# LUP-LuftbildUmweltPlanung/UNet

Hardware: AMD Instinct MI355X
Metric: 512x512 tiles/sec fwd+bwd (4-ch->5-class U-Net) (higher is better)
Workload: dtype f32

## Files before the change

### include/unet_hip.h

```cpp
#ifndef UNET_HIP_H
#define UNET_HIP_H

#include <stddef.h>
#include <stdint.h>

#ifdef __cplusplus
extern "C" {
#endif

#define UNET_OK 0
#define UNET_E_BADARG (-1)
#define UNET_E_UNSUPPORTED (-2)
#define UNET_E_HIP (-3)

#define UNET_ABI_VERSION 8

int unet_abi_version(void);
const char* unet_last_error(void);

#define UNET_F32 0
#define UNET_BF16 1
typedef uint16_t unet_bf16;

typedef struct {
    int conv_splitk;
    int mfma_shape;
    int f32_big_tile;
    int bf16_big_tile;
    int t256_tiles_per_wg;
    int t256_sliver;
    int conv1x1_gemm;
    int wgrad_mfma_shape;
    int wgrad_bf16_k4;
    int wgrad_1x1;
    int wgrad_narrow;
    int plan_batch;
    int wgrad_wgs;
    int conv_smallcin;
    int conv_head1x1;
} unet_tuning;
void unet_tuning_default(unet_tuning* t);


#define UNET_CONV_RELU 1
#define UNET_CONV_MASK 4

#define UNET_CONV_FWD 0
#define UNET_CONV_DGRAD 1

typedef struct {
    const float* x; int x_cs, x_co;
    const float* wp;
    const float* bias;
    const float* res; int res_cs, res_co;
    const float* mask; int mask_cs, mask_co;
    float* y; int y_cs, y_co;
    int N, IH, IW, Cin;
    int OH, OW, Cout;
    int ks, stride;
    int kind, flags;
    float* colsum;
    float* colsumsq;
// ... 21 lines not shown
int unet_pack_weights_bf16(const float* w, unet_bf16* wp, int Cout, int Cin, int ks, int mode, void* stream);
typedef struct {
    const float* w;
    void* wp;
    int Cout, Cin, ks, mode;
    const float* out_scale;
} unet_pack_job;
size_t unet_pack_batch_table_bytes(int njobs);
int unet_pack_batch_build(const unet_pack_job* jobs, int njobs, int dtype, void* table_host, unsigned* total_blocks);
int unet_pack_batch_run(const void* table_dev, int njobs, unsigned total_blocks, int dtype, void* stream);
typedef struct {
    const float* x; int x_cs, x_co;
    const float* dy; int dy_cs, dy_co;
    float* dw;
    float* dbias;
    int N, IH, IW, Cin, OH, OW, Cout, ks, stride;
    float* workspace; size_t workspace_floats;
    int accumulate;
    int dtype;
    const unet_tuning* tuning;
} unet_wgrad_desc;
size_t unet_conv2d_wgrad_workspace(const unet_wgrad_desc* d);
int unet_conv2d_wgrad_dma(const unet_wgrad_desc* d);
int unet_conv2d_wgrad(const unet_wgrad_desc* d, void* stream);

int unet_bn_stats_rows(long long P);
int unet_bn_stats(const float* x, int x_cs, int x_co, long long P, int C, float* partial, void* stream);
int unet_bn_finalize(const float* psum, const float* psumsq, int rows, long long count, int C,
                     const float* gamma, const float* beta, float* running_mean, float* running_var,
                     float momentum, float eps,
                     float* scale, float* shift, float* save_mean, float* save_invstd, long long* batches_tracked, void* stream);
int unet_bn_eval_coeffs(const float* gamma, const float* beta, const float* running_mean, const float* running_var,
                        float eps, int C, float* scale, float* shift, void* stream);
int unet_affine_act(const float* x, int x_cs, int x_co, const float* scale, const float* shift,
                    const float* x2, int x2_cs, int x2_co, const float* scale2, const float* shift2,
                    float* y, int y_cs, int y_co, long long P, int C, int relu, void* stream);
int unet_bn_bwd_reduce(const float* dout, int d_cs, int d_co, const float* out, int o_cs, int o_co,
                       const float* x, int x_cs, int x_co, const float* mean, const float* invstd,
                       long long P, int C, float* partial, void* stream);
int unet_bn_bwd_finalize(const float* partial, int rows, long long count, int C,
                         float* dgamma, float* dbeta, float* c1, float* c2, void* stream);
int unet_bn_bwd_apply(const float* dout, int d_cs, int d_co, const float* out, int o_cs, int o_co,
                      const float* x, int x_cs, int x_co, const float* mean, const float* invstd,
                      const float* gamma, const float* c1, const float* c2,
                      float* dx, int dx_cs, int dx_co, float* gout, int g_cs, int g_co, int g_accumulate,
                      long long P, int C, void* stream);
// ... 319 lines not shown
```

### unet_amd/_lib.py

```python
from __future__ import annotations

import ctypes as C
import os
import re
from pathlib import Path

import torch

_HERE = Path(__file__).resolve().parent
LIB_PATH = _HERE / "lib" / "libunet_hip.so"
HEADER = _HERE.parent / "include" / "unet_hip.h"

UNET_OK = 0
CONV_RELU = 1
CONV_MASK = 4
CONV_FWD = 0
CONV_DGRAD = 1
F32 = 0
BF16 = 1

c_float_p = C.POINTER(C.c_float)
vp = C.c_void_p


class Tuning(C.Structure):
    _fields_ = [(n, C.c_int) for n in ("conv_splitk", "mfma_shape", "f32_big_tile", "bf16_big_tile", "t256_tiles_per_wg", "t256_sliver",
                                       "conv1x1_gemm", "wgrad_mfma_shape", "wgrad_bf16_k4", "wgrad_1x1", "wgrad_narrow", "plan_batch", "wgrad_wgs", "conv_smallcin", "conv_head1x1")]

    @classmethod
    def default(cls, **over) -> "Tuning":
        t = cls()
        lib.unet_tuning_default(C.byref(t))
        for k, v in over.items():
            if k not in dict(cls._fields_):
                raise KeyError(f"unet_tuning has no field {k!r}")
            setattr(t, k, int(v))
        return t


class ConvDesc(C.Structure):
    _fields_ = [
        ("x", vp), ("x_cs", C.c_int), ("x_co", C.c_int),
        ("wp", vp),
        ("bias", vp),
        ("res", vp), ("res_cs", C.c_int), ("res_co", C.c_int),
        ("mask", vp), ("mask_cs", C.c_int), ("mask_co", C.c_int),
        ("y", vp), ("y_cs", C.c_int), ("y_co", C.c_int),
        ("N", C.c_int), ("IH", C.c_int), ("IW", C.c_int), ("Cin", C.c_int),
        ("OH", C.c_int), ("OW", C.c_int), ("Cout", C.c_int),
        ("ks", C.c_int), ("stride", C.c_int),
# ... 85 lines not shown


lib = _load()

i, ll, f, sz = C.c_int, C.c_longlong, C.c_float, C.c_size_t
_sig = {
    "unet_abi_version": (i, []),
    "unet_last_error": (C.c_char_p, []),
    "unet_conv2d_colsum_rows": (i, [C.POINTER(ConvDesc)]),
    "unet_conv2d": (i, [C.POINTER(ConvDesc), vp]),
    "unet_conv2d_variant": (i, [C.POINTER(ConvDesc)]),
    "unet_conv2d_splitk_workspace": (sz, [C.POINTER(ConvDesc)]),
    "unet_tuning_default": (None, [C.POINTER(Tuning)]),
    "unet_pack_batch_table_bytes": (sz, [i]),
    "unet_pack_batch_build": (i, [C.POINTER(PackJob), i, i, vp, C.POINTER(C.c_uint)]),
    "unet_pack_batch_run": (i, [vp, i, C.c_uint, i, vp]),
    "unet_pack_weights_size": (sz, [i, i, i, i]),
    "unet_pack_weights": (i, [vp, vp, i, i, i, i, vp]),
    "unet_pack_weights_strided": (i, [vp, ll, ll, vp, i, i, vp]),
    "unet_row_softmax": (i, [vp, i, i, vp, i, i, ll, i, vp]),
    "unet_row_softmax_bwd": (i, [vp, i, i, vp, i, i, vp, i, i, ll, i, vp]),
    "unet_conv2d_wgrad_workspace": (sz, [C.POINTER(WgradDesc)]),
    "unet_conv2d_wgrad_dma": (i, [C.POINTER(WgradDesc)]),
    "unet_conv2d_wgrad": (i, [C.POINTER(WgradDesc), vp]),
    "unet_bn_stats_rows": (i, [ll]),
    "unet_bn_stats": (i, [vp, i, i, ll, i, vp, vp]),
    "unet_bn_finalize": (i, [vp, vp, i, ll, i, vp, vp, vp, vp, f, f, vp, vp, vp, vp, vp, vp]),
    "unet_bn_eval_coeffs": (i, [vp, vp, vp, vp, f, i, vp, vp, vp]),
    "unet_affine_act": (i, [vp, i, i, vp, vp, vp, i, i, vp, vp, vp, i, i, ll, i, i, vp]),
    "unet_bn_bwd_reduce": (i, [vp, i, i, vp, i, i, vp, i, i, vp, vp, ll, i, vp, vp]),
    "unet_bn_bwd_finalize": (i, [vp, i, ll, i, vp, vp, vp, vp, vp]),
    "unet_bn_bwd_apply": (i, [vp, i, i, vp, i, i, vp, i, i, vp, vp, vp, vp, vp, vp, i, i, vp, i, i, i, ll, i, vp]),
    "unet_maxpool3x3s2": (i, [vp, i, i, vp, i, i, vp, i, i, i, i, i, i, vp]),
    "unet_maxpool3x3s2_bwd": (i, [vp, i, i, vp, vp, i, i, i, i, i, i, i, i, i, vp]),
    "unet_avgpool2_ceil": (i, [vp, i, i, vp, i, i, i, i, i, i, i, i, vp]),
    "unet_avgpool2_ceil_bwd": (i, [vp, i, i, vp, i, i, i, i, i, i, i, i, i, vp]),
    "unet_shuffle_blur": (i, [vp, i, i, vp, i, i, i, i, i, i, i, vp]),
    "unet_shuffle_blur_bwd": (i, [vp, i, i, vp, i, i, vp, i, i, i, i, i, i, i, vp]),
    "unet_shuffle_bwd_xmask": (i, [vp, i, i, vp, i, i, vp, i, i, i, i, i, i, vp]),
    "unet_resize_nearest": (i, [vp, i, i, vp, i, i, i, i, i, i, i, i, vp]),
    "unet_resize_nearest_bwd": (i, [vp, i, i, vp, i, i, i, i, i, i, i, i, vp]),
    "unet_nchw_to_nhwc": (i, [vp, vp, i, i, i, i, i, i, vp]),
    "unet_nhwc_to_nchw": (i, [vp, i, i, vp, i, i, i, i, vp]),
    "unet_copy_slice": (i, [vp, i, i, vp, i, i, ll, i, i, vp]),
    "unet_relu_mask": (i, [vp, i, i, vp, i, i, vp, i, i, ll, i, vp]),
    "unet_colsum": (i, [vp, i, i, ll, i, vp, vp, vp]),
# ... 146 lines not shown
```

### unet_amd/csrc/conv_dispatch.hip

```cpp
#include <stdlib.h>

#include "conv_common.h"

namespace unetconv {
static int env_int(const char* name, int dflt) {
    const char* e = getenv(name);
    return (e != nullptr && e[0] != 0) ? atoi(e) : dflt;
}
const unet_tuning& tuning_defaults() {
    static const unet_tuning t = [] {
        unet_tuning v;
        v.conv_splitk = env_int("UNET_CONV_SPLITK", 1);
        v.mfma_shape = 16;
        v.f32_big_tile = 1;
        v.bf16_big_tile = 1;
        v.t256_tiles_per_wg = 0;
        v.t256_sliver = env_int("UNET_T256_SLIVER", 1);
        v.conv1x1_gemm = env_int("UNET_CONV1X1_GEMM", 0);
        v.wgrad_mfma_shape = 32;
        v.wgrad_bf16_k4 = 1;
        v.wgrad_1x1 = 1;
        v.wgrad_narrow = 1;
        v.plan_batch = 0;
        v.wgrad_wgs = env_int("UNET_WGRAD_WGS", 0);
        v.conv_smallcin = env_int("UNET_CONV_SMALLCIN", 1);
        v.conv_head1x1 = env_int("UNET_CONV_HEAD1X1", 1);
        return v;
    }();
    return t;
}
}

extern "C" void unet_tuning_default(unet_tuning* t) {
    if (t != nullptr) *t = unetconv::tuning_defaults();
}

namespace {

using namespace unetconv;

int make_plan(const unet_conv_desc* d, Plan* p, int kc, int vec, int mf, int big_tile, int splitk, int plan_batch) {
    UNET_CHECK_ARG(d != nullptr, "conv: null desc");
    UNET_CHECK_ARG(d->x && d->wp && d->y, "conv: null tensor pointer");
    UNET_CHECK_ARG(d->ks == 1 || d->ks == 3, "conv: ks must be 1 or 3 (got %d)", d->ks);
    UNET_CHECK_ARG(d->stride == 1 || d->stride == 2, "conv: stride must be 1 or 2 (got %d)", d->stride);
    UNET_CHECK_ARG(!(d->ks == 1 && d->stride != 1), "conv: 1x1 stride 2 unsupported");
    UNET_CHECK_ARG(d->N > 0 && d->IH > 0 && d->IW > 0 && d->OH > 0 && d->OW > 0 && d->Cin > 0 && d->Cout > 0, "conv: bad dims");
    UNET_CHECK_ARG(unet::slice_ok_v(d->x_cs, d->x_co, d->Cin, vec), "conv: bad x slice cs=%d co=%d C=%d", d->x_cs, d->x_co, d->Cin);
    UNET_CHECK_ARG(unet::slice_ok_v(d->y_cs, d->y_co, d->Cout, d->y_f32 ? 4 : vec), "conv: bad y slice cs=%d co=%d C=%d", d->y_cs, d->y_co, d->Cout);
// ... 278 lines not shown
```

### unet_amd/csrc/conv_wgrad.hip

```cpp

#include <type_traits>
#include <utility>

#include "common.h"
#include "wgrad_plan.h"

namespace {

template <typename F, int... Is>
__device__ __forceinline__ void static_for_impl(F&& f, std::integer_sequence<int, Is...>) { (f(std::integral_constant<int, Is>{}), ...); }
template <int N, typename F>
__device__ __forceinline__ void static_for(F&& f) { static_for_impl(f, std::make_integer_sequence<int, N>{}); }


typedef float f32x16 __attribute__((ext_vector_type(16)));

constexpr int BK = 64;
constexpr int BC = 64;

struct WArgs {
    const float* x; const float* dy; float* part;
    float* bpart;
    int x_cs, x_co, dy_cs, dy_co;
    int N, IH, IW, Cin, Cin4, OH, OW, Cout, Cout4;
// ... 119 lines not shown
                        acc[r * KS + s] = __builtin_amdgcn_mfma_f32_32x32x2f32(av, bv, acc[r * KS + s], 0, 0, 0);
                    }
            }
            }
            __builtin_amdgcn_sched_barrier(0);
        });
        __syncthreads();
        if (has_next) store_tile();
        __syncthreads();
    }

    if (do_bias) {
        reinterpret_cast<float4*>(smem)[tid] = bq4;
        __syncthreads();
        if (tid < BK && k0 + tid < a.Cout) {
            float t = 0.f;
#pragma unroll
            for (int rr = 0; rr < 16; ++rr) t += smem[rr * 64 + tid];
            a.bpart[(size_t)split * a.Cout + k0 + tid] = t;
        }
    }
    const size_t KC_ = (size_t)a.Cout * a.Cin;
    float* pb = a.part + ((size_t)split * nsub + sub) * T * KC_;
    const int c = c0 + wc * 32 + l31;
#pragma unroll
    for (int t = 0; t < T; ++t)
#pragma unroll
        for (int r = 0; r < 16; ++r) {
            const int k = k0 + wk * 32 + (r & 3) + 8 * (r >> 2) + 4 * h;
            if (k < a.Cout && c < a.Cin) pb[(size_t)t * KC_ + (size_t)k * a.Cin + c] = acc[t][r];
        }
}

template <int PTW, int S, int KS>
__global__ __launch_bounds__(256, 2) void wgrad16_kernel(const WArgs a) {
    constexpr int PT = (S == 1) ? 64 : 32;
    constexpr int PTH = PT / PTW;
    constexpr int PAD = (KS - 1) / 2;
    constexpr int T = KS * KS;
    constexpr int HH = (PTH - 1) * S + KS, HW = (PTW - 1) * S + KS, HPIX = HH * HW;
    constexpr int DIT = (PT * 16 + 255) / 256;
    constexpr int XIT = (HPIX * 16 + 255) / 256;
    typedef float f32x4 __attribute__((ext_vector_type(4)));
    constexpr int LD = (S == 1) ? 80 : 72;

    extern __shared__ __attribute__((aligned(16))) float smem[];
// ... 938 lines not shown
        __syncthreads();
        if (tid < 128 && k0 + tid < a.Cout) {
            float t = 0.f;
#pragma unroll
            for (int rr = 0; rr < 8; ++rr) t += smem[rr * 128 + tid];
            a.bpart[(size_t)split * a.Cout + k0 + tid] = t;
        }
    }
    const size_t KC_ = (size_t)a.Cout * a.Cin;
    float* pb = a.part + (size_t)split * KC_;
#pragma unroll
    for (int i = 0; i < 2; ++i)
#pragma unroll
        for (int j = 0; j < 2; ++j) {
            const int c = c0 + wc * 64 + 32 * j + l31;
#pragma unroll
            for (int r = 0; r < 16; ++r) {
                const int k = k0 + wk * 64 + 32 * i + (r & 3) + 8 * (r >> 2) + 4 * h;
                if (k < a.Cout && c < a.Cin) pb[(size_t)k * a.Cin + c] = acc[i][j][r];
            }
        }
}

template <int K4>
__global__ __launch_bounds__(256) void wgrad1x1_small_kernel(const WArgs a, long long P, int PS, long long pix_per_block) {
    extern __shared__ __attribute__((aligned(16))) float smem[];
    const int C4 = a.Cin4 >> 2;
    const int tid = threadIdx.x;
    const int q = tid % C4, lane = tid / C4;
    const bool active = lane < PS;
    const long long p_begin = (long long)blockIdx.x * pix_per_block;
    long long p_end = p_begin + pix_per_block;
    if (p_end > P) p_end = P;
    float acc[4 * K4][4];
    float bsum[4 * K4];
#pragma unroll
    for (int k = 0; k < 4 * K4; ++k) {
        bsum[k] = 0.f;
#pragma unroll
        for (int j = 0; j < 4; ++j) acc[k][j] = 0.f;
    }
    if (active) {
        for (long long p = p_begin + lane; p < p_end; p += PS) {
            const float4 xv = *reinterpret_cast<const float4*>(a.x + (size_t)p * a.x_cs + a.x_co + 4 * q);
            const float* dyp = a.dy + (size_t)p * a.dy_cs + a.dy_co;
#pragma unroll
// ... 111 lines not shown
        const size_t t = e / KC_, i = e - t * KC_;
        float* o = dw + i * T + t;
        *o = accumulate ? (*o + s) : s;
    }
}

__global__ __launch_bounds__(256) void wgrad_bias_reduce_kernel(const float* __restrict__ bpart, float* __restrict__ dbias, int splits, int Cout) {
    __shared__ double part[4][64];
    const int cl = threadIdx.x & 63, q = threadIdx.x >> 6;
    const int c = blockIdx.x * 64 + cl;
    double s = 0.0;
    if (c < Cout)
        for (int sp = q; sp < splits; sp += 4) s += (double)bpart[(size_t)sp * Cout + c];
    part[q][cl] = s;
    __syncthreads();
    if (q == 0 && c < Cout) dbias[c] = (float)(((part[0][cl] + part[1][cl]) + part[2][cl]) + part[3][cl]);
}

struct WPlan {
    unet_tuning tune;
    WArgs k;
    int ptw, splits, T, narrow, gemm1x1, small1x1, ps, bf16;
    int dma;
    int nsub;
    long long pix_per_block;
    size_t lds_bytes, lds_bytes16;
};

int make_wplan(const unet_wgrad_desc* d, WPlan* p, bool need_dw = true) {
    UNET_CHECK_ARG(d != nullptr, "wgrad: null desc");
    p->tune = unetconv::tuning_of(d->tuning);
    UNET_CHECK_ARG(p->tune.wgrad_mfma_shape == 16 || p->tune.wgrad_mfma_shape == 32, "wgrad: unet_tuning.wgrad_mfma_shape must be 16 or 32 (start from unet_tuning_default())");
    UNET_CHECK_ARG(d->x && d->dy && (d->dw || !need_dw), "wgrad: null tensor pointer");
    UNET_CHECK_ARG(d->ks == 1 || d->ks == 3, "wgrad: ks must be 1 or 3");
    UNET_CHECK_ARG(d->stride == 1 || d->stride == 2, "wgrad: stride must be 1 or 2");
    UNET_CHECK_ARG(!(d->ks == 1 && d->stride != 1), "wgrad: 1x1 stride 2 unsupported");
    UNET_CHECK_ARG(d->N > 0 && d->IH > 0 && d->IW > 0 && d->OH > 0 && d->OW > 0 && d->Cin > 0 && d->Cout > 0, "wgrad: bad dims");
    UNET_CHECK_ARG((long long)d->N * d->OH * d->OW < (1ll << 31), "wgrad: more than 2^31 output pixels");
    const int pad = (d->ks - 1) / 2;
    UNET_CHECK_ARG(d->OH == (d->IH + 2 * pad - d->ks) / d->stride + 1 && d->OW == (d->IW + 2 * pad - d->ks) / d->stride + 1,
                   "wgrad: output dims inconsistent");
    UNET_CHECK_ARG(d->dtype == UNET_F32 || d->dtype == UNET_BF16, "wgrad: unknown dtype %d", d->dtype);
    const int vec = d->dtype == UNET_BF16 ? 8 : 4;
    p->bf16 = d->dtype == UNET_BF16;
    UNET_CHECK_ARG(unet::slice_ok_v(d->x_cs, d->x_co, d->Cin, vec), "wgrad: bad x slice");
    UNET_CHECK_ARG(unet::slice_ok_v(d->dy_cs, d->dy_co, d->Cout, vec), "wgrad: bad dy slice");
    UNET_CHECK_ARG(unet::aligned16(d->x) && unet::aligned16(d->dy), "wgrad: x/dy must be 16-byte aligned");
    WArgs& k = p->k;
    memset(&k, 0, sizeof(k));
    k.x = d->x; k.dy = d->dy; k.part = d->workspace;
    k.x_cs = d->x_cs; k.x_co = d->x_co; k.dy_cs = d->dy_cs; k.dy_co = d->dy_co;
    k.N = d->N; k.IH = d->IH; k.IW = d->IW; k.Cin = d->Cin; k.Cin4 = unet::roundup(d->Cin, vec);
    k.OH = d->OH; k.OW = d->OW; k.Cout = d->Cout; k.Cout4 = unet::roundup(d->Cout, vec);
    p->T = d->ks * d->ks;
    p->nsub = 1;
    p->dma = 0;
    p->ptw = d->OW >= 32 ? 32 : (d->OW >= 16 ? 16 : 8);
    const int pt = p->bf16 ? (d->stride == 1 ? 128 : 32) : (d->stride == 1 ? 64 : 32);
    const int pth = pt / p->ptw;
    k.tiles_y = unet::cdiv(d->OH, pth);
    k.tiles_x = unet::cdiv(d->OW, p->ptw);
    k.total_tiles = d->N * k.tiles_y * k.tiles_x;
    k.kt = unet::cdiv(d->Cout, BK);
    k.ct = unet::cdiv(d->Cin, BC);
    p->narrow = (!p->bf16 && p->tune.wgrad_narrow && d->ks == 3 && d->stride == 1 && d->Cout > 80 && d->Cout <= 112 && d->OW >= 32) ? 1 : 0;
    int cols = k.kt * k.ct;
    if (p->narrow) {
        p->ptw = 32;
        k.tiles_y = d->OH;
        k.tiles_x = unet::cdiv(d->OW, 32);
        k.total_tiles = d->N * k.tiles_y * k.tiles_x;
        const int nch = unet::cdiv(d->Cin, 112);
        k.cw = unet::roundup(unet::cdiv(d->Cin, nch), 4);
        const int ntw = d->Cout > 96 ? 5 : 7;
        k.nnb = unet::cdiv(unet::cdiv(9 * k.cw, 16), 4 * ntw);
        cols = nch * k.nnb;
        p->dma = p->tune.wgrad_narrow != 4 && flat_dma_fits(d->Cin, k.cw, k.nnb, ntw) && (long long)d->IW * d->x_cs * 4 < (1ll << 31) &&
                 (long long)d->OW * d->dy_cs * 4 < (1ll << 31);
    }
// ... 24 lines not shown
    if (p->gemm1x1) {
        k.kt = unet::cdiv(d->Cout, 128);
        k.ct = unet::cdiv(d->Cin, 128);
        k.total_tiles = unet::cdiv((long long)d->N * d->OH * d->OW, 64);
        k.tiles_y = k.tiles_x = 1;
        cols = k.kt * k.ct;
    }
    int target = 512;
    if (p->tune.wgrad_wgs > 0) target = p->tune.wgrad_wgs;
    else if (p->bf16 && d->ks == 3 && d->stride == 1 && (long long)k.total_tiles * cols <= 20000) target = 256;
    int want = target / cols;
    if ((p->narrow || p->bf16) && want >= 8) want &= ~7;
    if (want < 1) want = 1;
    int tpb = unet::cdiv(k.total_tiles, want);
    if (tpb < 4) tpb = 4;
    if (tpb > k.total_tiles) tpb = k.total_tiles;
    k.tiles_per_block = tpb;
    p->splits = unet::cdiv(k.total_tiles, tpb);
    if (!p->bf16 && !p->narrow && !p->gemm1x1 && p->tune.wgrad_mfma_shape == 32 && p->tune.wgrad_narrow != 3) {
        k.csub = d->Cin <= 32 ? 1 : 0;
        k.ksub = d->Cout <= 32 ? 1 : 0;
        p->nsub = (1 + k.csub) * (1 + k.ksub);
    }
    const int hh = (pth - 1) * d->stride + d->ks, hw = (p->ptw - 1) * d->stride + d->ks;
    p->lds_bytes = (size_t)(pt * BK + hh * hw * BC) * sizeof(float);
    p->lds_bytes16 = (size_t)(pt + hh * hw) * (d->stride == 1 ? 80 : 72) * sizeof(float);
    if (p->bf16) p->lds_bytes = (size_t)pt * 160 + (size_t)hh * hw * (d->stride == 1 ? 160 : 144);
    return UNET_OK;
}


template <int PTW, int S, int KS>
int launch_w16(const WPlan& p, hipStream_t st) {
    auto kern = wgrad16_kernel<PTW, S, KS>;
    static unsigned long long configured = 0;
    if (unet::first_use_on_device(&configured)) {
        UNET_CHECK_HIP(hipFuncSetAttribute((const void*)kern, hipFuncAttributeMaxDynamicSharedMemorySize, 160 * 1024));
    }
    hipLaunchKernelGGL(kern, dim3(p.k.kt * p.k.ct, p.splits), dim3(256), p.lds_bytes16, st, p.k);
    UNET_CHECK_LAUNCH();
    return UNET_OK;
}

template <int PTW, int S, int KS>
int launch_w(const WPlan& p, hipStream_t st) {
    if (p.tune.wgrad_mfma_shape == 16) return launch_w16<PTW, S, KS>(p, st);
// ... 59 lines not shown
    if (stride == 1) return launch_wb<PTW, 1, 3>(p, st);
    return launch_wb<PTW, 2, 3>(p, st);
}

template <int PTW>
int launch_w_ptw(const WPlan& p, int ks, int stride, hipStream_t st) {
    if (ks == 1) return launch_w<PTW, 1, 1>(p, st);
    if (stride == 1) return launch_w<PTW, 1, 3>(p, st);
    return launch_w<PTW, 2, 3>(p, st);
}

}

extern "C" size_t unet_conv2d_wgrad_workspace(const unet_wgrad_desc* d) {
    WPlan p;
    if (make_wplan(d, &p) != UNET_OK) return 0;
    return (size_t)p.splits * p.nsub * p.T * d->Cout * d->Cin + (size_t)p.splits * d->Cout;
}

extern "C" int unet_conv2d_wgrad_dma(const unet_wgrad_desc* d) {
    WPlan p;
    if (make_wplan(d, &p, false) != UNET_OK) return -1;
    return p.dma;
}

extern "C" int unet_conv2d_wgrad(const unet_wgrad_desc* d, void* stream) {
    WPlan p;
    int rc = make_wplan(d, &p);
    if (rc != UNET_OK) return rc;
    const size_t npart = (size_t)p.splits * p.nsub * p.T * d->Cout * d->Cin;
    const size_t need = npart + (size_t)p.splits * d->Cout;
    UNET_CHECK_ARG(d->workspace != nullptr && d->workspace_floats >= need, "wgrad: workspace too small (%zu < %zu floats)",
                   d->workspace_floats, need);
    p.k.bpart = d->dbias != nullptr ? d->workspace + npart : nullptr;
    hipStream_t st = (hipStream_t)stream;
    if (p.bf16) {
        switch (p.ptw) {
            case 32: rc = launch_wb_ptw<32>(p, d->ks, d->stride, st); break;
            case 16: rc = launch_wb_ptw<16>(p, d->ks, d->stride, st); break;
            default: rc = launch_wb_ptw<8>(p, d->ks, d->stride, st); break;
        }
    } else if (p.small1x1) {
        const long long P = (long long)d->N * d->OH * d->OW;
        const dim3 grid((unsigned)p.splits);
        const int k4 = (d->Cout + 3) / 4;
        const size_t lds = (size_t)p.ps * (4 * k4 * p.k.Cin4 + 4 * k4) * sizeof(float);
        UNET_CHECK_ARG(lds <= 64 * 1024, "wgrad: head kernel needs %zu bytes of LDS", lds);
        switch (k4) {
            case 1: hipLaunchKernelGGL(wgrad1x1_small_kernel<1>, grid, dim3(256), lds, st, p.k, P, p.ps, p.pix_per_block); break;
            case 2: hipLaunchKernelGGL(wgrad1x1_small_kernel<2>, grid, dim3(256), lds, st, p.k, P, p.ps, p.pix_per_block); break;
            case 3: hipLaunchKernelGGL(wgrad1x1_small_kernel<3>, grid, dim3(256), lds, st, p.k, P, p.ps, p.pix_per_block); break;
            default: hipLaunchKernelGGL(wgrad1x1_small_kernel<4>, grid, dim3(256), lds, st, p.k, P, p.ps, p.pix_per_block); break;
        }
        UNET_CHECK_LAUNCH();
        rc = UNET_OK;
    } else if (p.gemm1x1) {
        static unsigned long long configured = 0;
        if (unet::first_use_on_device(&configured)) {
            UNET_CHECK_HIP(hipFuncSetAttribute((const void*)wgrad1x1_kernel, hipFuncAttributeMaxDynamicSharedMemorySize, 160 * 1024));
        }
        hipLaunchKernelGGL(wgrad1x1_kernel, dim3(p.k.kt * p.k.ct, p.splits), dim3(256), (size_t)2 * 64 * 128 * sizeof(float), st, p.k,
                           (long long)d->N * d->OH * d->OW);
        UNET_CHECK_LAUNCH();
        rc = UNET_OK;
    } else if (p.narrow) {
        const size_t lds = p.dma ? (size_t)(2 * 32 * 112 + 3 * 15 * 256) * sizeof(float)
                                 : (size_t)(32 + 3 * 34) * 112 * sizeof(float) + (size_t)4 * 256 * 16;
        const dim3 grid(unet::cdiv(d->Cin, p.k.cw) * p.k.nnb, unet::roundup(p.splits, 8));
        static unsigned long long configured = 0;
        if (unet::first_use_on_device(&configured)) {
            UNET_CHECK_HIP(hipFuncSetAttribute((const void*)wgrad_flat_kernel<7, 5>, hipFuncAttributeMaxDynamicSharedMemorySize, 160 * 1024));
            UNET_CHECK_HIP(hipFuncSetAttribute((const void*)wgrad_flat_kernel<6, 5, true>, hipFuncAttributeMaxDynamicSharedMemorySize, 160 * 1024));
            UNET_CHECK_HIP(hipFuncSetAttribute((const void*)wgrad_flat_kernel<6, 7>, hipFuncAttributeMaxDynamicSharedMemorySize, 160 * 1024));
            UNET_CHECK_HIP(hipFuncSetAttribute((const void*)wgrad_flat_kernel<7, 5, false, true>, hipFuncAttributeMaxDynamicSharedMemorySize, 160 * 1024));
            UNET_CHECK_HIP(hipFuncSetAttribute((const void*)wgrad_flat_kernel<6, 5, true, true>, hipFuncAttributeMaxDynamicSharedMemorySize, 160 * 1024));
            UNET_CHECK_HIP(hipFuncSetAttribute((const void*)wgrad_flat_kernel<6, 7, false, true>, hipFuncAttributeMaxDynamicSharedMemorySize, 160 * 1024));
        }
        const bool sliver = d->Cout > 96 && d->Cout <= 100 && p.tune.wgrad_narrow != 2;
        if (p.dma) {
            if (sliver) hipLaunchKernelGGL((wgrad_flat_kernel<6, 5, true, true>), grid, dim3(256), lds, st, p.k);
            else if (d->Cout > 96) hipLaunchKernelGGL((wgrad_flat_kernel<7, 5, false, true>), grid, dim3(256), lds, st, p.k);
            else hipLaunchKernelGGL((wgrad_flat_kernel<6, 7, false, true>), grid, dim3(256), lds, st, p.k);
        } else if (sliver) hipLaunchKernelGGL((wgrad_flat_kernel<6, 5, true>), grid, dim3(256), lds, st, p.k);
        else if (d->Cout > 96) hipLaunchKernelGGL((wgrad_flat_kernel<7, 5>), grid, dim3(256), lds, st, p.k);
        else hipLaunchKernelGGL((wgrad_flat_kernel<6, 7>), grid, dim3(256), lds, st, p.k);
        UNET_CHECK_LAUNCH();
        rc = UNET_OK;
    } else
    switch (p.ptw) {
        case 32: rc = launch_w_ptw<32>(p, d->ks, d->stride, st); break;
        case 16: rc = launch_w_ptw<16>(p, d->ks, d->stride, st); break;
        default: rc = launch_w_ptw<8>(p, d->ks, d->stride, st); break;
    }
    if (rc != UNET_OK) return rc;
    const size_t KC_ = (size_t)d->Cout * d->Cin;
    const int slices = p.splits * p.nsub;
    if (p.small1x1)
        hipLaunchKernelGGL(wgrad_reduce_rows_kernel, dim3(unet::cdiv((int)(KC_ * p.T), 64)), dim3(256), 0, st, d->workspace, d->dw,
                           p.splits, p.T, KC_, d->accumulate);
    else if (slices >= 32 && KC_ * p.T < ((size_t)1 << 31) / 8)
        hipLaunchKernelGGL(wgrad_reduce_q_kernel<8>, dim3((unsigned)unet::cdiv((long long)(KC_ * p.T), 32LL)), dim3(256), 0, st, d->workspace, d->dw,
                           slices, p.T, KC_, d->accumulate);
    else if (slices >= 8 && KC_ * p.T < ((size_t)1 << 31) / 8)
        hipLaunchKernelGGL(wgrad_reduce_q_kernel<4>, dim3((unsigned)unet::cdiv((long long)(KC_ * p.T), 64LL)), dim3(256), 0, st, d->workspace, d->dw,
                           slices, p.T, KC_, d->accumulate);
    else
        hipLaunchKernelGGL(wgrad_reduce_kernel, dim3(unet::ew_grid((long long)KC_ * p.T, 256)), dim3(256), 0, st, d->workspace, d->dw,
                           slices, p.T, KC_, d->accumulate);
// ... 9 lines not shown
```

### unet_amd/csrc/wgrad_plan.h

```cpp
#pragma once

inline bool flat_dma_fits(int Cin, int cw, int nnb, int ntw) {
    const int nch = (Cin + cw - 1) / cw;
    const int widths[2] = {nch > 1 ? cw : Cin, Cin - (nch - 1) * cw};
    for (int CW : widths)
        for (int nb = 0; nb < nnb; ++nb) {
            const int lo = nb * 64 * ntw;
            int hi = lo + 64 * ntw;
            if (hi > 9 * CW) hi = 9 * CW;
            if (lo >= hi) continue;
            if ((hi - 1) / (3 * CW) - lo / (3 * CW) > 1) return false;
        }
    return true;
}
```

### unet_amd/ops.py

```python
from __future__ import annotations

import ctypes as C
import math
from dataclasses import dataclass
from typing import Optional

import torch

from . import _lib as L
from ._lib import ConvDesc, WgradDesc, check, lib


import contextlib
import threading

_TUNE = threading.local()


@contextlib.contextmanager
def tuning(**fields):
    prev = getattr(_TUNE, "cur", None)
    cur = L.Tuning.default() if prev is None else L.Tuning.from_buffer_copy(prev)
    for k, v in fields.items():
        if k not in dict(L.Tuning._fields_):
# ... 433 lines not shown
    d.N, d.IH, d.IW, d.Cin = x.N, x.H, x.W, x.C
    d.OH, d.OW, d.Cout = dy.H, dy.W, dy.C
    d.ks, d.stride = ks, stride
    d.workspace = _p(ws)
    d.workspace_floats = 0 if ws is None else ws.numel()
    d.accumulate = int(accumulate)
    d.tuning = _tuning_ptr()
    assert x.bf16 == dy.bf16
    d.dtype = L.BF16 if x.bf16 else L.F32
    return d


def wgrad_workspace(x: TS, dy: TS, ks, stride, with_bias=False) -> int:
    d = _wgrad_desc(x, dy, torch.empty(0), None, ks, stride, None, 0)
    d.dw = 1
    return int(lib.unet_conv2d_wgrad_workspace(C.byref(d)))


def wgrad_uses_dma(x: TS, dy: TS, ks, stride) -> bool:
    d = _wgrad_desc(x, dy, None, None, ks, stride, None, 0)
    r = lib.unet_conv2d_wgrad_dma(C.byref(d))
    assert r >= 0, "wgrad_uses_dma: bad descriptor"
    return r == 1


def conv2d_wgrad(x: TS, dy: TS, dw: torch.Tensor, ks: int, stride: int, ws: torch.Tensor, dbias=None, accumulate=False):
    d = _wgrad_desc(x, dy, dw, dbias, ks, stride, ws, accumulate)
    check(lib.unet_conv2d_wgrad(C.byref(d), _stream()), "conv2d_wgrad")



def bn_stats_rows(P: int) -> int:
    return lib.unet_bn_stats_rows(P)


def bn_stats(x: TS, partial: torch.Tensor):
    check(_fn("bn_stats", x)(x.ptr, x.cs, x.co, x.P, x.C, partial.data_ptr(), _stream()), "bn_stats")


def bn_finalize(psum, psumsq, rows, count, C_, gamma, beta, rmean, rvar, momentum, eps, scale, shift, smean, sinvstd, tracked=None):
    assert tracked is None or tracked.dtype == torch.int64
    check(lib.unet_bn_finalize(_p(psum), _p(psumsq), rows, count, C_, _p(gamma), _p(beta), _p(rmean), _p(rvar), momentum, eps,
                               _p(scale), _p(shift), _p(smean), _p(sinvstd), _p(tracked), _stream()), "bn_finalize")


def bn_eval_coeffs(gamma, beta, rmean, rvar, eps, scale, shift):
# ... 1522 lines not shown
```

Baseline: 150.9.

## Add LDS-DMA double-buffered wgrad kernels for general 3x3 and 1x1 cases

Adds two weight-gradient kernels that use buffer_load_lds direct-to-LDS DMA with double buffering. The 3x3 stride-1 kernel streams rows through a 7-slot ring and processes two output rows per unit. The 1x1 GEMM kernel uses 32-pixel stages. Both are on by default via a new tuning flag and are selected when the shapes fit. The aim is to overlap global loads with MFMA work and drop register staging. In exchange they use more LDS, add new code paths and per-row barriers, and can route shapes away from the tuned flat kernels.

```diff
diff --git a/include/unet_hip.h b/include/unet_hip.h
--- a/include/unet_hip.h
+++ b/include/unet_hip.h
@@ -38,6 +38,7 @@
     int wgrad_wgs;
     int conv_smallcin;
     int conv_head1x1;
+    int wgrad_general_dma;
 } unet_tuning;
 void unet_tuning_default(unet_tuning* t);
 
@@ -105,6 +106,7 @@
 } unet_wgrad_desc;
 size_t unet_conv2d_wgrad_workspace(const unet_wgrad_desc* d);
 int unet_conv2d_wgrad_dma(const unet_wgrad_desc* d);
+int unet_conv2d_wgrad_form(const unet_wgrad_desc* d);
 int unet_conv2d_wgrad(const unet_wgrad_desc* d, void* stream);
 
 int unet_bn_stats_rows(long long P);
diff --git a/unet_amd/_lib.py b/unet_amd/_lib.py
--- a/unet_amd/_lib.py
+++ b/unet_amd/_lib.py
@@ -25,7 +25,7 @@
 
 class Tuning(C.Structure):
     _fields_ = [(n, C.c_int) for n in ("conv_splitk", "mfma_shape", "f32_big_tile", "bf16_big_tile", "t256_tiles_per_wg", "t256_sliver",
-                                       "conv1x1_gemm", "wgrad_mfma_shape", "wgrad_bf16_k4", "wgrad_1x1", "wgrad_narrow", "plan_batch", "wgrad_wgs", "conv_smallcin", "conv_head1x1")]
+                                       "conv1x1_gemm", "wgrad_mfma_shape", "wgrad_bf16_k4", "wgrad_1x1", "wgrad_narrow", "plan_batch", "wgrad_wgs", "conv_smallcin", "conv_head1x1", "wgrad_general_dma")]
 
     @classmethod
     def default(cls, **over) -> "Tuning":
@@ -157,6 +157,7 @@
     "unet_row_softmax_bwd": (i, [vp, i, i, vp, i, i, vp, i, i, ll, i, vp]),
     "unet_conv2d_wgrad_workspace": (sz, [C.POINTER(WgradDesc)]),
     "unet_conv2d_wgrad_dma": (i, [C.POINTER(WgradDesc)]),
+    "unet_conv2d_wgrad_form": (i, [C.POINTER(WgradDesc)]),
     "unet_conv2d_wgrad": (i, [C.POINTER(WgradDesc), vp]),
     "unet_bn_stats_rows": (i, [ll]),
     "unet_bn_stats": (i, [vp, i, i, ll, i, vp, vp]),
diff --git a/unet_amd/csrc/conv_dispatch.hip b/unet_amd/csrc/conv_dispatch.hip
--- a/unet_amd/csrc/conv_dispatch.hip
+++ b/unet_amd/csrc/conv_dispatch.hip
@@ -25,6 +25,7 @@
         v.wgrad_wgs = env_int("UNET_WGRAD_WGS", 0);
         v.conv_smallcin = env_int("UNET_CONV_SMALLCIN", 1);
         v.conv_head1x1 = env_int("UNET_CONV_HEAD1X1", 1);
+        v.wgrad_general_dma = env_int("UNET_WGRAD_GENERAL_DMA", 1);
         return v;
     }();
     return t;
diff --git a/unet_amd/csrc/conv_wgrad.hip b/unet_amd/csrc/conv_wgrad.hip
--- a/unet_amd/csrc/conv_wgrad.hip
+++ b/unet_amd/csrc/conv_wgrad.hip
@@ -165,6 +165,170 @@
     }
     const size_t KC_ = (size_t)a.Cout * a.Cin;
     float* pb = a.part + ((size_t)split * nsub + sub) * T * KC_;
+    const int c = c0 + wc * 32 + l31;
+#pragma unroll
+    for (int t = 0; t < T; ++t)
+#pragma unroll
+        for (int r = 0; r < 16; ++r) {
+            const int k = k0 + wk * 32 + (r & 3) + 8 * (r >> 2) + 4 * h;
+            if (k < a.Cout && c < a.Cin) pb[(size_t)t * KC_ + (size_t)k * a.Cin + c] = acc[t][r];
+        }
+}
+
+__global__ __launch_bounds__(256, 2) void wgrad_rows_dma_kernel(const WArgs a) {
+    constexpr int PT = 32, HW = 34, T = 9, NS = 7;
+    constexpr int DYT = PT * BK;
+    constexpr int SLOT = 9 * 256;
+    constexpr int DIT = 2, RIT = 3;
+    extern __shared__ __attribute__((aligned(16))) float smem[];
+    float* dyT = smem;
+    float* ring = smem + 2 * DYT;
+
+    const int tid = threadIdx.x, lane = tid & 63, wave = __builtin_amdgcn_readfirstlane(tid >> 6);
+    const int wk = wave >> 1, wc = wave & 1;
+    const int l31 = lane & 31, h = lane >> 5;
+    const int kblk = blockIdx.x / a.ct, cblk = blockIdx.x % a.ct;
+    const int k0 = kblk * BK, c0 = cblk * BC;
+    const int split = blockIdx.y;
+    const int tile_begin = split * a.tiles_per_block;
+    int tile_end = tile_begin + a.tiles_per_block;
+    if (tile_end > a.total_tiles) tile_end = a.total_tiles;
+
+    f32x16 acc[T];
+#pragma unroll
+    for (int t = 0; t < T; ++t)
+#pragma unroll
+        for (int r = 0; r < 16; ++r) acc[t][r] = 0.f;
+
+    typedef __attribute__((address_space(3))) void* lds_ptr;
+    constexpr unsigned OOB = 0x80000000u;
+    const int dy_row_b = (a.OW * a.dy_cs - a.dy_co - k0) * 4, x_row_b = (a.IW * a.x_cs - a.x_co - c0) * 4;
+    unsigned dvo[DIT], xvo[RIT];
+    auto unit_setup = [&](int ox0) {
+#pragma unroll
+        for (int it = 0; it < DIT; ++it) {
+            const int e = tid + it * 256;
+            const int p = e >> 4, q = e & 15;
+            const bool ok = (ox0 + p) < a.OW && (k0 + 4 * q) < a.Cout4;
+            dvo[it] = ok ? (unsigned)((ox0 + p) * a.dy_cs + 4 * q) * 4u : OOB;
+        }
+#pragma unroll
+        for (int j = 0; j < RIT; ++j) {
+            const int e = tid + j * 256;
+            const int hx = e >> 4, q = e & 15;
+            const int ix = ox0 - 1 + hx;
+            const bool ok = (e < HW * 16) && ix >= 0 && ix < a.IW && (c0 + 4 * q) < a.Cin4;
+            xvo[j] = ok ? (unsigned)(ix * a.x_cs + 4 * q) * 4u : OOB;
+        }
+    };
+    auto dma_dy = [&](int img, int oy, int buf) {
+        const float* row = a.dy + ((size_t)img * a.OH + oy) * a.OW * a.dy_cs + a.dy_co + k0;
+        const __amdgpu_buffer_rsrc_t rs = __builtin_amdgcn_make_buffer_rsrc(const_cast<float*>(row), 0, dy_row_b, 0x00020000);
+        float* dst = dyT + buf * DYT + wave * 256;
+#pragma unroll
+        for (int it = 0; it < DIT; ++it) __builtin_amdgcn_raw_ptr_buffer_load_lds(rs, (lds_ptr)(dst + it * 1024), 16, (int)dvo[it], 0, 0, 0);
+    };
+    auto slot_of = [&](int s) { return s >= NS ? s - NS : s; };
+    auto dma_row = [&](int img, int iy, int slot) {
+        const bool rowok = iy >= 0 && iy < a.IH;
+        const float* row = a.x + ((size_t)img * a.IH + (rowok ? iy : 0)) * a.IW * a.x_cs + a.x_co + c0;
+        const __amdgpu_buffer_rsrc_t rs = __builtin_amdgcn_make_buffer_rsrc(const_cast<float*>(row), 0, rowok ? x_row_b : 0, 0x00020000);
+        float* dst = ring + slot * SLOT + wave * 256;
+#pragma unroll
+        for (int j = 0; j < RIT; ++j)
+            if (j * 256 + wave * 64 < HW * 16)
+                __builtin_amdgcn_raw_ptr_buffer_load_lds(rs, (lds_ptr)(dst + j * 1024), 16, (int)xvo[j], 0, 0, 0);
+    };
+    auto land_and_meet = [&]() { asm volatile("s_waitcnt vmcnt(0) lgkmcnt(0)\n\ts_barrier" ::: "memory"); };
+    auto unit_pos = [&](int u, int& img, int& oy0, int& ox0) {
+        int b = u;
+        ox0 = (b % a.tiles_x) * PT; b /= a.tiles_x;
+        oy0 = (b % a.tiles_y) * 2;
+        img = b / a.tiles_y;
+    };
+    auto fetch_unit = [&](int img, int oy0, int ox0, int b, int buf) {
+        unit_setup(ox0);
+        dma_dy(img, oy0, buf);
+        for (int r = 0; r < 3; ++r) dma_row(img, oy0 - 1 + r, slot_of(b + r));
+    };
+    const bool do_bias = a.bpart != nullptr && cblk == 0;
+    float4 bq4 = make_float4(0.f, 0.f, 0.f, 0.f);
+    auto bias_add_tile = [&](int buf) {
+        const float4* src = reinterpret_cast<const float4*>(dyT + buf * DYT) + tid;
+#pragma unroll
+        for (int it = 0; it < DIT; ++it) {
+            const float4 v = src[it * 256];
+            bq4.x += v.x; bq4.y += v.y; bq4.z += v.z; bq4.w += v.w;
+        }
+    };
+    const int aoff = h * BK + wk * 32 + l31, boff = h * BC + wc * 32 + l31;
+    auto mma_tile = [&](int s0, int buf) {
+        const float* ab = dyT + buf * DYT + aoff;
+        const float* br[3];
+#pragma unroll
+        for (int r = 0; r < 3; ++r) br[r] = ring + slot_of(s0 + r) * SLOT + boff;
+        static_for<4>([&](auto g) {
+            constexpr int G = decltype(g)::value;
+#pragma unroll
+            for (int sg = 0; sg < 4; ++sg) {
+                const int step = G * 4 + sg;
+                const float av = ab[(2 * step) * BK];
+#pragma unroll
+                for (int r = 0; r < 3; ++r)
+#pragma unroll
+                    for (int s = 0; s < 3; ++s) {
+                        const float bv = br[r][(2 * step + s) * BC];
+                        acc[r * 3 + s] = __builtin_amdgcn_mfma_f32_32x32x2f32(av, bv, acc[r * 3 + s], 0, 0, 0);
+                    }
+            }
+            __builtin_amdgcn_sched_barrier(0);
+        });
+    };
+
+    if (tile_begin < tile_end) {
+        int img, oy0, ox0;
+        int b = 0, cur = 0;
+        unit_pos(tile_begin, img, oy0, ox0);
+        fetch_unit(img, oy0, ox0, 0, 0);
+        land_and_meet();
+        for (int u = tile_begin; u < tile_end; ++u) {
+            const bool two = oy0 + 1 < a.OH;
+            const bool has_next = u + 1 < tile_end;
+            int nimg = img, noy0 = oy0, nox0 = ox0;
+            if (has_next) unit_pos(u + 1, nimg, noy0, nox0);
+            if (do_bias) bias_add_tile(cur);
+            if (two) { dma_dy(img, oy0 + 1, cur ^ 1); dma_row(img, oy0 + 2, slot_of(b + 3)); }
+            else if (has_next) fetch_unit(nimg, noy0, nox0, slot_of(b + 4), cur ^ 1);
+            mma_tile(b, cur);
+            if (two) {
+                land_and_meet();
+                cur ^= 1;
+                if (do_bias) bias_add_tile(cur);
+                if (has_next) fetch_unit(nimg, noy0, nox0, slot_of(b + 4), cur ^ 1);
+                mma_tile(slot_of(b + 1), cur);
+            }
+            if (has_next) {
+                land_and_meet();
+                cur ^= 1;
+                b = slot_of(b + 4);
+                img = nimg; oy0 = noy0; ox0 = nox0;
+            }
+        }
+    }
+
+    if (do_bias) {
+        __syncthreads();
+        reinterpret_cast<float4*>(smem)[tid] = bq4;
+        __syncthreads();
+        if (tid < BK && k0 + tid < a.Cout) {
+            float t = 0.f;
+#pragma unroll
+            for (int rr = 0; rr < 16; ++rr) t += smem[rr * 64 + tid];
+            a.bpart[(size_t)split * a.Cout + k0 + tid] = t;
+        }
+    }
+    const size_t KC_ = (size_t)a.Cout * a.Cin;
+    float* pb = a.part + (size_t)split * T * KC_;
     const int c = c0 + wc * 32 + l31;
 #pragma unroll
     for (int t = 0; t < T; ++t)
@@ -1149,6 +1313,117 @@
         }
 }
 
+__global__ __launch_bounds__(256, 2) void wgrad1x1_dma_kernel(const WArgs a, long long P) {
+    constexpr int SP = 32, LDW = 128, IT = SP * 32 / 256;
+    constexpr int STG = 2 * SP * LDW;
+    extern __shared__ __attribute__((aligned(16))) float smem[];
+
+    const int tid = threadIdx.x, lane = tid & 63, wave = __builtin_amdgcn_readfirstlane(tid >> 6);
+    const int wk = wave >> 1, wc = wave & 1;
+    const int l31 = lane & 31, h = lane >> 5;
+    const int kblk = blockIdx.x / a.ct, cblk = blockIdx.x % a.ct;
+    const int k0 = kblk * 128, c0 = cblk * 128;
+    const int split = blockIdx.y;
+    const long long tile_begin = (long long)split * a.tiles_per_block;
+    long long tile_end = tile_begin + a.tiles_per_block;
+    if (tile_end > a.total_tiles) tile_end = a.total_tiles;
+
+    f32x16 acc[2][2];
+#pragma unroll
+    for (int i = 0; i < 2; ++i)
+#pragma unroll
+        for (int j = 0; j < 2; ++j)
+#pragma unroll
+            for (int r = 0; r < 16; ++r) acc[i][j][r] = 0.f;
+
+    typedef __attribute__((address_space(3))) void* lds_ptr;
+    constexpr unsigned OOB = 0x80000000u;
+    unsigned dvo[IT], xvo[IT];
+#pragma unroll
+    for (int it = 0; it < IT; ++it) {
+        const int e = tid + it * 256;
+        const int p = e >> 5, q = e & 31;
+        dvo[it] = (k0 + 4 * q) < a.Cout4 ? (unsigned)(p * a.dy_cs + 4 * q) * 4u : OOB;
+        xvo[it] = (c0 + 4 * q) < a.Cin4 ? (unsigned)(p * a.x_cs + 4 * q) * 4u : OOB;
+    }
+    auto dma_stage = [&](long long p0, int buf) {
+        const long long left = P - p0;
+        const int npix = left >= SP ? SP : (left > 0 ? (int)left : 0);
+        const long long pb = npix > 0 ? p0 : 0;
+        const __amdgpu_buffer_rsrc_t rd_ = __builtin_amdgcn_make_buffer_rsrc(const_cast<float*>(a.dy) + (size_t)pb * a.dy_cs + a.dy_co + k0, 0,
+                                                                             npix > 0 ? (npix * a.dy_cs - a.dy_co - k0) * 4 : 0, 0x00020000);
+        const __amdgpu_buffer_rsrc_t rx_ = __builtin_amdgcn_make_buffer_rsrc(const_cast<float*>(a.x) + (size_t)pb * a.x_cs + a.x_co + c0, 0,
+                                                                             npix > 0 ? (npix * a.x_cs - a.x_co - c0) * 4 : 0, 0x00020000);
+        float* dst = smem + buf * STG + wave * 256;
+#pragma unroll
+        for (int it = 0; it < IT; ++it) {
+            __builtin_amdgcn_raw_ptr_buffer_load_lds(rd_, (lds_ptr)(dst + it * 1024), 16, (int)dvo[it], 0, 0, 0);
+            __builtin_amdgcn_raw_ptr_buffer_load_lds(rx_, (lds_ptr)(dst + SP * LDW + it * 1024), 16, (int)xvo[it], 0, 0, 0);
+        }
+    };
+    auto land_and_meet = [&]() { asm volatile("s_waitcnt vmcnt(0) lgkmcnt(0)\n\ts_barrier" ::: "memory"); };
+    const bool do_bias = a.bpart != nullptr && cblk == 0;
+    float4 bq4 = make_float4(0.f, 0.f, 0.f, 0.f);
+    auto bias_add_stage = [&](int buf) {
+        const float4* src = reinterpret_cast<const float4*>(smem + buf * STG) + tid;
+#pragma unroll
+        for (int it = 0; it < IT; ++it) {
+            const float4 v = src[it * 256];
+            bq4.x += v.x; bq4.y += v.y; bq4.z += v.z; bq4.w += v.w;
+        }
+    };
+    const int aoff = h * LDW + wk * 64 + l31, boff = SP * LDW + h * LDW + wc * 64 + l31;
+
+    const long long nstage = 2 * (tile_end - tile_begin);
+    if (nstage > 0) {
+        const long long pbeg = tile_begin * 64;
+        int cur = 0;
+        dma_stage(pbeg, 0);
+        land_and_meet();
+        for (long long s = 0; s < nstage; ++s) {
+            if (do_bias) bias_add_stage(cur);
+            if (s + 1 < nstage) dma_stage(pbeg + (s + 1) * SP, cur ^ 1);
+            const float* ab = smem + cur * STG + aoff;
+            const float* bb = smem + cur * STG + boff;
+#pragma unroll
+            for (int step = 0; step < SP / 2; ++step) {
+                const float a0 = ab[(2 * step) * LDW], a1 = ab[(2 * step) * LDW + 32];
+                const float b0 = bb[(2 * step) * LDW], b1 = bb[(2 * step) * LDW + 32];
+                acc[0][0] = __builtin_amdgcn_mfma_f32_32x32x2f32(a0, b0, acc[0][0], 0, 0, 0);
+                acc[0][1] = __builtin_amdgcn_mfma_f32_32x32x2f32(a0, b1, acc[0][1], 0, 0, 0);
+                acc[1][0] = __builtin_amdgcn_mfma_f32_32x32x2f32(a1, b0, acc[1][0], 0, 0, 0);
+                acc[1][1] = __builtin_amdgcn_mfma_f32_32x32x2f32(a1, b1, acc[1][1], 0, 0, 0);
+            }
+            land_and_meet();
+            cur ^= 1;
+        }
+    }
+
+    if (do_bias) {
+        reinterpret_cast<float4*>(smem)[tid] = bq4;
+        __syncthreads();
+        if (tid < 128 && k0 + tid < a.Cout) {
+            float t = 0.f;
+#pragma unroll
+            for (int rr = 0; rr < 8; ++rr) t += smem[rr * 128 + tid];
+            a.bpart[(size_t)split * a.Cout + k0 + tid] = t;
+        }
+    }
+    const size_t KC_ = (size_t)a.Cout * a.Cin;
+    float* pb = a.part + (size_t)split * KC_;
+#pragma unroll
+    for (int i = 0; i < 2; ++i)
+#pragma unroll
+        for (int j = 0; j < 2; ++j) {
+            const int c = c0 + wc * 64 + 32 * j + l31;
+#pragma unroll
+            for (int r = 0; r < 16; ++r) {
+                const int k = k0 + wk * 64 + 32 * i + (r & 3) + 8 * (r >> 2) + 4 * h;
+                if (k < a.Cout && c < a.Cin) pb[(size_t)k * a.Cin + c] = acc[i][j][r];
+            }
+        }
+}
+
 template <int K4>
 __global__ __launch_bounds__(256) void wgrad1x1_small_kernel(const WArgs a, long long P, int PS, long long pix_per_block) {
     extern __shared__ __attribute__((aligned(16))) float smem[];
@@ -1306,6 +1581,8 @@
     WArgs k;
     int ptw, splits, T, narrow, gemm1x1, small1x1, ps, bf16;
     int dma;
+    int gdma;
+    int sdma;
     int nsub;
     long long pix_per_block;
     size_t lds_bytes, lds_bytes16;
@@ -1339,6 +1616,8 @@
     p->T = d->ks * d->ks;
     p->nsub = 1;
     p->dma = 0;
+    p->sdma = 0;
+    p->gdma = 0;
     p->ptw = d->OW >= 32 ? 32 : (d->OW >= 16 ? 16 : 8);
     const int pt = p->bf16 ? (d->stride == 1 ? 128 : 32) : (d->stride == 1 ? 64 : 32);
     const int pth = pt / p->ptw;
@@ -1409,6 +1688,9 @@
         k.ksub = d->Cout <= 32 ? 1 : 0;
         p->nsub = (1 + k.csub) * (1 + k.ksub);
     }
+    p->gdma = (p->gemm1x1 && p->tune.wgrad_general_dma != 0 && gemm1x1_dma_fits(d->x_cs, d->dy_cs)) ? 1 : 0;
+    p->sdma = (!p->bf16 && !p->narrow && p->tune.wgrad_general_dma != 0 &&
+               general_dma_fits(d->ks, d->stride, d->IW, d->OW, d->x_cs, d->dy_cs, d->Cin, d->Cout, p->tune.wgrad_mfma_shape)) ? 1 : 0;
     const int hh = (pth - 1) * d->stride + d->ks, hw = (p->ptw - 1) * d->stride + d->ks;
     p->lds_bytes = (size_t)(pt * BK + hh * hw * BC) * sizeof(float);
     p->lds_bytes16 = (size_t)(pt + hh * hw) * (d->stride == 1 ? 80 : 72) * sizeof(float);
@@ -1514,6 +1796,12 @@
     WPlan p;
     if (make_wplan(d, &p, false) != UNET_OK) return -1;
     return p.dma;
+}
+
+extern "C" int unet_conv2d_wgrad_form(const unet_wgrad_desc* d) {
+    WPlan p;
+    if (make_wplan(d, &p, false) != UNET_OK) return -1;
+    return p.dma ? 1 : (p.sdma ? 2 : (p.gdma ? 3 : 0));
 }
 
 extern "C" int unet_conv2d_wgrad(const unet_wgrad_desc* d, void* stream) {
@@ -1550,9 +1838,14 @@
         static unsigned long long configured = 0;
         if (unet::first_use_on_device(&configured)) {
             UNET_CHECK_HIP(hipFuncSetAttribute((const void*)wgrad1x1_kernel, hipFuncAttributeMaxDynamicSharedMemorySize, 160 * 1024));
-        }
-        hipLaunchKernelGGL(wgrad1x1_kernel, dim3(p.k.kt * p.k.ct, p.splits), dim3(256), (size_t)2 * 64 * 128 * sizeof(float), st, p.k,
-                           (long long)d->N * d->OH * d->OW);
+            UNET_CHECK_HIP(hipFuncSetAttribute((const void*)wgrad1x1_dma_kernel, hipFuncAttributeMaxDynamicSharedMemorySize, 160 * 1024));
+        }
+        if (p.gdma)
+            hipLaunchKernelGGL(wgrad1x1_dma_kernel, dim3(p.k.kt * p.k.ct, p.splits), dim3(256), (size_t)2 * 2 * 32 * 128 * sizeof(float), st, p.k,
+                               (long long)d->N * d->OH * d->OW);
+        else
+            hipLaunchKernelGGL(wgrad1x1_kernel, dim3(p.k.kt * p.k.ct, p.splits), dim3(256), (size_t)2 * 64 * 128 * sizeof(float), st, p.k,
+                               (long long)d->N * d->OH * d->OW);
         UNET_CHECK_LAUNCH();
         rc = UNET_OK;
     } else if (p.narrow) {
@@ -1576,6 +1869,13 @@
         } else if (sliver) hipLaunchKernelGGL((wgrad_flat_kernel<6, 5, true>), grid, dim3(256), lds, st, p.k);
         else if (d->Cout > 96) hipLaunchKernelGGL((wgrad_flat_kernel<7, 5>), grid, dim3(256), lds, st, p.k);
         else hipLaunchKernelGGL((wgrad_flat_kernel<6, 7>), grid, dim3(256), lds, st, p.k);
+        UNET_CHECK_LAUNCH();
+        rc = UNET_OK;
+    } else if (p.sdma) {
+        static unsigned long long configured = 0;
+        if (unet::first_use_on_device(&configured))
+            UNET_CHECK_HIP(hipFuncSetAttribute((const void*)wgrad_rows_dma_kernel, hipFuncAttributeMaxDynamicSharedMemorySize, 160 * 1024));
+        hipLaunchKernelGGL(wgrad_rows_dma_kernel, dim3(p.k.kt * p.k.ct, p.splits), dim3(256), (size_t)(2 * 32 * 64 + 7 * 9 * 256) * sizeof(float), st, p.k);
         UNET_CHECK_LAUNCH();
         rc = UNET_OK;
     } else
diff --git a/unet_amd/csrc/wgrad_plan.h b/unet_amd/csrc/wgrad_plan.h
--- a/unet_amd/csrc/wgrad_plan.h
+++ b/unet_amd/csrc/wgrad_plan.h
@@ -13,3 +13,13 @@
         }
     return true;
 }
+
+inline bool general_dma_fits(int ks, int stride, int IW, int OW, int x_cs, int dy_cs, int Cin, int Cout, int mfma_shape) {
+    if (ks != 3 || stride != 1 || OW < 32 || mfma_shape != 32) return false;
+    if (Cin <= 32 || Cout <= 32) return false;
+    return (long long)IW * x_cs * 4 < (1ll << 31) && (long long)OW * dy_cs * 4 < (1ll << 31);
+}
+
+inline bool gemm1x1_dma_fits(int x_cs, int dy_cs) {
+    return 32ll * x_cs * 4 < (1ll << 31) && 32ll * dy_cs * 4 < (1ll << 31);
+}
diff --git a/unet_amd/ops.py b/unet_amd/ops.py
--- a/unet_amd/ops.py
+++ b/unet_amd/ops.py
@@ -479,6 +479,13 @@
     r = lib.unet_conv2d_wgrad_dma(C.byref(d))
     assert r >= 0, "wgrad_uses_dma: bad descriptor"
     return r == 1
+
+
+def wgrad_form(x: TS, dy: TS, ks, stride) -> int:
+    d = _wgrad_desc(x, dy, None, None, ks, stride, None, 0)
+    r = lib.unet_conv2d_wgrad_form(C.byref(d))
+    assert r >= 0, "wgrad_form: bad descriptor"
+    return int(r)
 
 
 def conv2d_wgrad(x: TS, dy: TS, dw: torch.Tensor, ks: int, stride: int, ws: torch.Tensor, dbias=None, accumulate=False):
```

New measurement: 151.9, median of 6. No clear change (+0.7%).
